# underactuated/HSLabs

Measured on AMD Instinct MI355X. Metric: batched control-loop steps/sec (hexapod.xml, 18-DoF) at 1/2/4/8 MI355X, higher is better.
Workload: dtype f64

## Files before the change

### hslabs_amd/api.py

```python
from __future__ import annotations

import ctypes
from dataclasses import dataclass, field

import numpy as np

from . import capi

GAIT_DTYPE = np.dtype([
    ("torso_pos", "<f8", (3,)), ("torso_angles", "<f8", (3,)), ("step_duration", "<f8"),
    ("period", "<f8"), ("step_length", "<f8"), ("step_height", "<f8"), ("curvature", "<f8"),
    ("foot_shift", "<f8"), ("foot_shift_type", "<i4"), ("rec_transform_flag", "<i4"),
    ("rec_transl", "<f8", (3,)), ("rec_eas", "<f8", (3,)), ("reserved", "<f8", (5,)),
])
assert GAIT_DTYPE.itemsize == 192


def _require(ok: bool, msg: str) -> None:
    if not ok:
        raise ValueError(msg)


def _torch_stream(device, stream):
    import torch
# ... 171 lines not shown
            pass


def limb_tile_launches() -> int:
    return int(capi.load().hs_limb_tile_launches())


def limb_tile_plan_launches() -> int:
    return int(capi.load().hs_limb_tile_plan_launches())


def limb_tile_loop_launches() -> int:
    return int(capi.load().hs_limb_tile_loop_launches())


def limb_launches() -> int:
    return int(capi.load().hs_limb_launches())


def limb_deferred() -> int:
    d = ctypes.c_int64()
    capi.check(capi.load().hs_limb_stats(None, ctypes.byref(d)), "hs_limb_stats")
    return int(d.value)


def params_array(params) -> np.ndarray:
    if isinstance(params, np.ndarray) and params.dtype == GAIT_DTYPE:
        return np.ascontiguousarray(params)
    arr = np.zeros(len(params), GAIT_DTYPE)
    for i, p in enumerate(params):
        arr[i] = p.to_record()
    return arr


def run_host(model: KinematicModel, params, n_t: int = 20, k0: int = 0, horizon: int | None = None,
             ignore_reach: bool = True, want=("q", "tau", "cf", "x", "flags", "work_cot")) -> dict:
    arr = params_array(params)
    B = len(arr)
    H = n_t if horizon is None else horizon
    shapes = _out_shapes(model, B, H)
    out = {k: np.zeros(shapes[k], np.uint32 if k == "flags" else np.float64) if k in want else None
           for k in ("q", "tau", "cf", "x", "flags", "work_cot")}
    dp = ctypes.POINTER(ctypes.c_double)

    def P(a, t=dp):
        return None if a is None else a.ctypes.data_as(t)
# ... 792 lines not shown
```

### hslabs_amd/capi.py

```python
from __future__ import annotations

import ctypes
import hashlib
import os

from . import build as _build

ABI_VERSION = 16

HS_OK = 0
HS_FLAG_RANK_RETRY = 1
HS_FLAG_FULL_RANK = 2
HS_FLAG_LOOP_EXHAUST = 4
HS_FLAG_NAN = 8
HS_FLAG_UNREACH = 16
HS_FLAG_NO_CONTACT = 32
HS_FLAG_GENERAL = 64
HS_FLAG_NEAR_RANK = 256
HS_FLAG_DEPENDENT = 512
HS_PREC_F64 = 0
HS_PREC_F32 = 1
HS_SOLVE_AUTO = 0
HS_SOLVE_REFERENCE = 1
KEY_MIN_STEP_LENGTH = 1e-3
COMM_ID_BYTES = 128

EXPORTS = [
    "hs_model_load", "hs_model_load_ex", "hs_model_free", "hs_model_get_dims", "hs_pgs_config_read",
    "hs_run", "hs_run_steps", "hs_run_calls", "hs_run_pd", "hs_run_forces", "hs_run_forces_calls", "hs_mixed_create", "hs_mixed_free",
    "hs_mixed_get_dims", "hs_complete_traj", "hs_traj_save", "hs_run_forces_host",
    "hs_run_mixed", "hs_run_mixed_steps", "hs_run_mixed_calls", "hs_run_host", "hs_best_key_cot", "hs_best_key_encode",
    "hs_best_key_decode", "hs_last_error", "hs_abi_version",
    "hs_sim_default_params", "hs_sim_reset", "hs_sim_step", "hs_sim_create", "hs_sim_advance", "hs_sim_get_state",
    "hs_sim_free", "hs_sim_trial", "hs_sim_trial_summary", "hs_sim_set_trial", "hs_sim_get_trial_state",
    "hs_sim_config", "hs_sim_track_push", "hs_sim_probe", "hs_sim_estimate_workspace",
    "hs_cpc_default_params", "hs_cpc_torques", "hs_cpc_target_points", "hs_sim_cpc_workspace", "hs_sim_cpc_step",
    "hs_batch_create", "hs_batch_set_params", "hs_batch_run", "hs_batch_run_device", "hs_select_best",
    "hs_batch_best_key_device", "hs_batch_free", "hs_comm_unique_id", "hs_comm_init", "hs_comm_free", "hs_comm_size",
    "hs_comm_reduce_best", "hs_select_best_comm", "hs_pergen_rec", "hs_pergen_rec_host", "hs_model_lik",
    "hs_model_lik_host", "hs_model_fk", "hs_model_fk_host", "hs_model_get_node", "hs_model_set_torso_penalty",
    "hs_model_get_torso_penalty", "hs_model_limb_lane", "hs_limb_launches", "hs_limb_tile_launches", "hs_limb_stats",
    "hs_limb_tile_plan_launches", "hs_limb_tile_loop_launches",
]
EXPORTS_B = ["hs_sim_regress_B", "hs_sim_estimate_B"]
HS_FLAG_LIK_FAILED = 128
SIM_BODY_STRIDE = 13
HS_TRIAL_RUNNING = -1
HS_TRIAL_SURVIVED = -2
HS_CPC_FLAG_NONFINITE = 1
HS_CPC_FLAG_NOSCORE = 2
HS_CPC_FLAG_RANK = 4


class GaitParamsC(ctypes.Structure):

    _fields_ = [
        ("torso_pos", ctypes.c_double * 3),
        ("torso_angles", ctypes.c_double * 3),
        ("step_duration", ctypes.c_double),
        ("period", ctypes.c_double),
        ("step_length", ctypes.c_double),
        ("step_height", ctypes.c_double),
        ("curvature", ctypes.c_double),
        ("foot_shift", ctypes.c_double),
        ("foot_shift_type", ctypes.c_int32),
# ... 236 lines not shown
    L.hs_batch_best_key_device.argtypes = [vp, ctypes.c_int32]
    L.hs_batch_best_key_device.restype = vp
    L.hs_batch_free.argtypes = [vp]
    L.hs_batch_free.restype = None
    u32p = ctypes.POINTER(ctypes.c_uint32)
    L.hs_pergen_rec.argtypes = [vp, vp, ctypes.c_int32, vp, ctypes.c_int32, vp, vp]
    L.hs_pergen_rec_host.argtypes = [vp, ctypes.POINTER(GaitParamsC), ctypes.c_int32, dp, ctypes.c_int32, dp]
    L.hs_model_lik.argtypes = [vp, ctypes.c_int32, vp, ctypes.c_int32, vp, vp, vp]
    L.hs_model_lik_host.argtypes = [vp, ctypes.c_int32, dp, ctypes.c_int32, dp, u32p]
    L.hs_model_fk.argtypes = [vp, ctypes.c_int32, vp, ctypes.c_int32, vp, vp, vp]
    L.hs_model_fk_host.argtypes = [vp, ctypes.c_int32, dp, ctypes.c_int32, dp, dp]
    L.hs_model_get_node.argtypes = [vp, ctypes.c_int32, ctypes.POINTER(NodeInfoC)]
    L.hs_last_error.argtypes = []
    L.hs_last_error.restype = ctypes.c_char_p
    L.hs_model_limb_lane.argtypes = [vp, ctypes.POINTER(ctypes.c_int32)]
    L.hs_limb_launches.argtypes = []
    L.hs_limb_launches.restype = ctypes.c_int64
    L.hs_limb_tile_launches.argtypes = []
    L.hs_limb_tile_launches.restype = ctypes.c_int64
    L.hs_limb_tile_plan_launches.argtypes = []
    L.hs_limb_tile_plan_launches.restype = ctypes.c_int64
    L.hs_limb_tile_loop_launches.argtypes = []
    L.hs_limb_tile_loop_launches.restype = ctypes.c_int64
    L.hs_limb_stats.argtypes = [ctypes.POINTER(ctypes.c_int64), ctypes.POINTER(ctypes.c_int64)]
    L.hs_abi_version.argtypes = []
    L.hs_abi_version.restype = ctypes.c_int
    if L.hs_abi_version() != ABI_VERSION:
        raise HSError("libhslabs ABI version mismatch")
    _lib = L
    return L


def check(rc: int, what: str = "") -> None:
    if rc != HS_OK:
        msg = load().hs_last_error().decode(errors="replace")
        raise HSError(f"{what}: {msg} (rc={rc})")
```

### hslabs_amd/csrc/hs_capi.cpp

```cpp
#include <hip/hip_runtime.h>

#include <algorithm>
#include <atomic>
#include <cmath>
#include <cstdio>
#include <cstdlib>
#include <cfloat>
#include <cstring>
#include <fstream>
#include <mutex>
#include <string>
#include <vector>

#include "hs_internal.h"

namespace {

thread_local std::string g_err;

int fail(int code, const std::string& msg) {
  g_err = msg;
  return code;
}

// ... 377 lines not shown
    std::lock_guard<std::mutex> lk(cx.pools->mu);
    hipError_t e = (hipError_t)cx.pools->fused_gen.get(
        a.stream, ((size_t)CHUNK * (B + 1) * hs::solve_workspace_bytes() + gwb - 1) / gwb, &gen);
    const size_t need = (size_t)S * B * sizeof(double);
    const size_t want =
        std::max(need, std::min((size_t)HS_FUSED_RESERVE_STEPS * B * sizeof(double), (size_t)512 << 20));
    if (e == hipSuccess) e = (hipError_t)cx.pools->fused_work.get(a.stream, (want + gwb - 1) / gwb, &work);
    if (e == hipSuccess)
      e = (hipError_t)cx.pools->fused_fix.get(a.stream, (fix_bytes(n_counts, CHUNK, mp) + gwb - 1) / gwb, &fix);
    if (e != hipSuccess) return hip_fail(e, "hipMalloc(fused workspace)");
  }
  int32_t* fix_counts = (int32_t*)fix;
  hs_run_args c = a;
  c.horizon = (int32_t)S;
  c.best_key = nullptr;
  hs_run_args r = a;
  if (r.key_steps == 0) r.key_steps = (int32_t)((int64_t)n_calls * a.horizon);
  mp.fused_h = a.horizon;
  mp.fused_work = work;
  mp.fused_gen = gen;
  fix_carve(fix, n_counts, mp);
  const bool barrier_ok = (B + 63) / 64 <= 1024 && env_switch("HS_FIX_BARRIER", true);
  mp.prep_unit = limb ? 8 : 2;
  int le = launch_setup(cx, c, mp);
  mp.red_total_mass = cx.total_mass;
  mp.red_rollout_mass = cx.rollout_mass;
  mp.red_key_steps = r.key_steps;
  hipStream_t st = (hipStream_t)a.stream;
  for (int32_t i = 0; le == 0 && i < n_chunks; i++) {
    const int64_t s0 = online ? 0 : (int64_t)i * CHUNK;
    const bool last = i + 1 == n_chunks;
    if (online) c.k0 = (int32_t)(((int64_t)a.k0 + (int64_t)i * a.horizon) % a.n_t);
    mp.fused_s0 = (int32_t)s0;
    mp.fused_n = (int32_t)std::min<int64_t>(CHUNK, S - s0);
    mp.fix_mode = hs::FIX_DEFER;
    mp.fix_count = fix_counts + i;
    mp.fix_reduce = 0;
    mp.limb_tile = limb_tile(rt, a, mp.fused_n);
    mp.limb_tile_loop = mp.limb_tile ? limb_tile_loop(a, mp.fused_n) : 1;
    hipError_t e = kernel_events ? hipEventRecord((hipEvent_t)kernel_events[2 * i], st) : hipSuccess;
    if (e != hipSuccess) return hip_fail(e, "hipEventRecord");
    int32_t planned = 0;
    le = limb ? k.launch_limb(cx.d_topo, c, cx.ws, mp, limb_tile_plan_mode(), &planned)
              : k.launch_fused(cx.d_topo, c, cx.ws, mp);
    g_limb_launches += limb;
    g_limb_tile_launches += mp.limb_tile;
// ... 36 lines not shown

int hs_abi_version(void) { return HSLABS_ABI_VERSION; }

int hs_model_limb_lane(hs_model_t m, int32_t* ok) {
  if (!m || !ok) return fail(HS_E_ARG, "null argument");
  *ok = m->host.limb_lane_ok;
  return HS_OK;
}

int64_t hs_limb_launches(void) { return g_limb_launches.load(); }
int64_t hs_limb_tile_launches(void) { return g_limb_tile_launches.load(); }
int64_t hs_limb_tile_plan_launches(void) { return g_limb_tile_plan_launches.load(); }
int64_t hs_limb_tile_loop_launches(void) { return g_limb_tile_loop_launches.load(); }

int hs_limb_stats(int64_t* launches, int64_t* deferred) {
  if (launches) *launches = g_limb_launches.load();
  if (deferred) {
    unsigned long long n[2] = {0, 0};
    hipError_t e = (hipError_t)hs::kernels_f64.limb_deferred(&n[0]);
    if (e == hipSuccess) e = (hipError_t)hs::kernels_f32.limb_deferred(&n[1]);
    if (e != hipSuccess) return hip_fail(e, "hs_limb_stats");
    *deferred = (int64_t)(n[0] + n[1]);
  }
  return HS_OK;
}

const char* hs_last_error(void) { return g_err.c_str(); }

int hs_model_load_ex(const char* xml_path, int lik_variant, hs_model_t* out) {
  if (!xml_path || !out) return fail(HS_E_ARG, "null argument");
  hs_model_s* m = new hs_model_s;
  memset(m->dev, 0, sizeof(m->dev));
  memset(m->sim_dev, 0, sizeof(m->sim_dev));
  memset(m->sim_dev_f32, 0, sizeof(m->sim_dev_f32));
  std::string err;
  int rc = hs::load_model_file(xml_path, lik_variant, &m->host, err, &m->sim);
  if (rc != HS_OK) {
    delete m;
    return fail(rc, err);
  }
  *out = m;
  return HS_OK;
}

int hs_model_load(const char* xml_path, hs_model_t* out) { return hs_model_load_ex(xml_path, -1, out); }

// ... 1597 lines not shown
```

### hslabs_amd/csrc/hs_internal.h

```cpp
#pragma once
#include <cstddef>
#include <mutex>
#include <string>
#include <vector>

#include "../../include/hslabs.h"
#include "hs_simtopo.h"
#include "hs_limb_tile.h"
#include "hs_topo.h"

struct hs_sim_probe_kargs {
  hs_sim_args sim;
  int32_t m, pad;
  const double* tau0;
  const double* dtau;
  double* config_out;
  double* tau_out;
  double* body_out;
  uint32_t* seed_out;
};

namespace hs {

int set_error(int code, const std::string& msg);
// ... 13 lines not shown
  int32_t n_waves;
  int32_t max_parts;
  int32_t h_row;
  int32_t setup_io;
  const double* tau_in;
  const double *pd_q, *pd_dq;
  double pd_k1, pd_k2;
  double *pd_tau, *pd_q0, *pd_dq0;
  int32_t st_tau, st_cf, st_q, st_x;
  int32_t fused_w, fused_s0, fused_n, fused_h;
  void* fused_work;
  void* fused_gen;
  int32_t setup_only;
  int32_t fix_mode;
  int32_t* fix_count;
  int32_t* fix_items;
  int32_t fix_n_counts;
  int32_t fix_reduce, red_key_steps, red_n_steps;
  int32_t* fix_barrier;
  double red_total_mass;
  const double* red_rollout_mass;
  uint64_t* red_best_key;
  int32_t ktab_n, ktab_lo, ktab_nl, ttab_n;
  int32_t prep_unit;
  const int32_t *limb_model, *limb_rollouts, *limb_slots;
  int32_t limb_waves;
  int32_t limb_tile;
  int32_t limb_tile_loop;
};

size_t solve_workspace_bytes();
void ktab_range(int32_t k0, int32_t n_t, int32_t horizon, int64_t n_calls, int32_t* lo, int32_t* n_table,
                int32_t* n_ttab);
launch_map single_model_map(const hs_topo& t, int32_t n_rollouts);

struct kernels {
  size_t (*general_workspace_bytes)();
  int (*launch_rollouts)(const hs_topo* d_topo, const hs_run_args& a, void* workspace, const launch_map& mp);
  int (*launch_fused)(const hs_topo* d_topo, const hs_run_args& a, void* workspace, const launch_map& mp);
  int (*launch_limb)(const hs_topo* d_topo, const hs_run_args& a, void* workspace, const launch_map& mp,
                     int32_t tile_plan, int32_t* tile_planned);
  int (*launch_fused_reduce)(const hs_run_args& a, double total_mass, const double* rollout_mass,
                             const void* work_steps, int32_t n_steps);
  int (*limb_deferred)(unsigned long long* out);
};
extern const kernels kernels_f64, kernels_f32;
inline const kernels& kernels_of(int32_t precision) { return precision == HS_PREC_F32 ? kernels_f32 : kernels_f64; }

int launch_pergen_rec(const hs_topo* d_topo, const hs_gait_params* params, int32_t n_rollouts, const double* times,
                      int32_t n_times, double* rec, void* stream);
int launch_fk(const hs_topo* d_topo, int32_t n_parts, int32_t n_cfg, const double* config, int32_t stride,
              double* a_ground, double* a_joint, void* stream);
int launch_lik(const hs_topo* d_topo, int32_t n_cfg, const double* rec, int32_t ignore_reach, double* config,
               uint32_t* status, void* stream);
// ... 65 lines not shown
```

### hslabs_amd/csrc/hs_kernels.hip

```cpp
#include "hs_rollout_kernel.h"
#include "hs_limb.h"

namespace {

__global__ __launch_bounds__(WAVE) void hs_pergen_rec_kernel(const hs_topo* __restrict__ T,
                                                             const hs_gait_params* __restrict__ params,
                                                             int32_t n_rollouts, const double* __restrict__ times,
                                                             int32_t n_times, double* __restrict__ rec) {
  __shared__ SetupL st[2];
  const int sub = threadIdx.x / HALF, lane = threadIdx.x % HALF;
  const int64_t n_items = (int64_t)n_rollouts * n_times;
  const int64_t item = (int64_t)blockIdx.x * 2 + sub;
  const bool live = item < n_items;
  const int64_t it = live ? item : n_items - 1;
  const int b = (int)(it / n_times), ti = (int)(it % n_times);
  const GaitR g = load_gait(params[b]);
  gait_setup(T, g, 1, st[sub], lane);
  const int nl = T->n_limbs;
  if (live && lane < nl) {
    real o0[3], o1[3], target[3];
    bool turned;
    gait_record<false>(g, params[b], limb_rec(st[sub], T->limb_pergen[lane]), (real)times[ti], o0, o1, turned, target);
    double* r = rec + it * (6 + 3 * nl);
    if (lane == 0)
// ... 13 lines not shown

#ifdef HS_STAMPS
extern "C" int hs_debug_read_stamps(unsigned long long* out, int n_rows) {
  if (n_rows > 4096) n_rows = 4096;
  return (int)hipMemcpyFromSymbol(out, HIP_SYMBOL(g_stamps), sizeof(unsigned long long) * 32 * n_rows, 0,
                                  hipMemcpyDeviceToHost);
}
extern "C" int hs_debug_set_stamp_base(unsigned int base) {
  return (int)hipMemcpyToSymbol(HIP_SYMBOL(g_stamp_base), &base, sizeof(base), 0, hipMemcpyHostToDevice);
}
extern "C" int hs_debug_set_stamp_iter(int iter) {
  return (int)hipMemcpyToSymbol(HIP_SYMBOL(g_stamp_iter), &iter, sizeof(iter), 0, hipMemcpyHostToDevice);
}
extern "C" int hs_debug_clear_stamps() {
  static unsigned long long zero[4096][32];
  return (int)hipMemcpyToSymbol(HIP_SYMBOL(g_stamps), zero, sizeof(zero), 0, hipMemcpyHostToDevice);
}
#endif

namespace hs {

size_t solve_workspace_bytes() { return sizeof(SolveWS); }

void ktab_range(int32_t k0, int32_t n_t, int32_t horizon, int64_t n_calls, int32_t* lo_out, int32_t* n_out,
                int32_t* ttab_out) {
  int64_t lo = INT64_MAX, hi = 0;
  const int64_t nc = n_calls < n_t ? n_calls : n_t;
  for (int64_t c = 0; c < nc; c++) {
    const int64_t f = ((int64_t)k0 + c * horizon) % n_t;
    lo = f < lo ? f : lo;
    hi = f + horizon + NS - 1 > hi ? f + horizon + NS - 1 : hi;
  }
  const int64_t n = nc > 0 ? hi - lo : 0;
  *lo_out = nc > 0 ? (int32_t)lo : 0;
  *n_out = n <= HS_KTAB ? (int32_t)n : 0;
  *ttab_out = (int32_t)(n < HS_KTAB ? n : HS_KTAB);
}

int launch_pergen_rec(const hs_topo* d_topo, const hs_gait_params* params, int32_t n_rollouts, const double* times,
                      int32_t n_times, double* rec, void* stream) {
  const int64_t items = (int64_t)n_rollouts * n_times;
  if (items <= 0) return 0;
  hipLaunchKernelGGL(hs_pergen_rec_kernel, dim3((unsigned)((items + 1) / 2)), dim3(WAVE), 0, (hipStream_t)stream,
                     d_topo, params, n_rollouts, times, n_times, rec);
  return (int)hipGetLastError();
}
// ... 8 lines not shown
```

### hslabs_amd/csrc/hs_limb.h

```cpp
#pragma once
#include "hs_limb_tile.h"
#include "hs_step_base.h"
#include "hs_step_kin.h"
#include "hs_step_solve.h"

namespace {

#ifndef HS_LIMB_WAVES
#define HS_LIMB_WAVES 2
#endif
#ifndef HS_LIMB_WAVES_F32
#define HS_LIMB_WAVES_F32 HS_LIMB_WAVES
#endif

constexpr int LG = 8;
constexpr int LGR = WAVE / LG;

__device__ inline int dbg_row(bool live, int b, int horizon, int s_glob) { return live ? b * horizon + s_glob : -1; }
#ifdef HS_DBG
#define LDBG(dbg_r, slot, val, n)                                                                                \
  do {                                                                                                           \
    if (HS_DBG == (n) && (dbg_r) >= 0 && (size_t)(dbg_r) * 32 + (slot) < (1u << 22)) g_dbg[(size_t)(dbg_r) * 32 + (slot)] = (double)(val); \
  } while (0)
#else
// ... 122 lines not shown
  return s;
}

__device__ __attribute__((always_inline)) inline A34 limb_frame(const hs_topo* T, int L, bool straight, const bool own,
                                                                const RolloutWS& W, const KinFrames& kf, int row,
                                                                const real* u, real tv, BodyS& ob) {
  if (straight) {
    if (own) ob = body_straight(kf.own[L][0], u, tv);
    return frame_at(load34r(kf.J0[L]), u, tv);
  }
  A34 A = load34r(W.ktor[row] + 6);
  const int clen = T->limb_chain_len[L];
  for (int kk = 1; kk < clen; kk++) {
    const int v = T->limb_chain[L][kk];
    A = mul(A, node_pj(T, v));
    if (T->node[v].owner_limb == L) {
      const real com[3] = {(real)T->node[v].com[0], (real)T->node[v].com[1], (real)T->node[v].com[2]};
      ob = body_frame(A, com);
    }
  }
  return mul(A, node_joint_parent(T, T->limb_child[L]));
}

__device__ inline bool sincos_big(real x) { return !(fabs(x) < (real)0x1p20); }
__device__ __attribute__((always_inline)) inline void limb_outer(const hs_topo* T, const hs_link (&LK)[3], const A34& J,
                                                                 const real* ja, real (&P)[3][3], real (&U)[3][3],
                                                                 bool& big) {
  real sq[3], cq[3];
#pragma unroll
  for (int kk = 0; kk < 3; kk++) {
    big |= sincos_big(ja[kk]);
    sincos_k_small(ja[kk], &sq[kk], &cq[kk]);
  }
  A34 Jv = J, H;
  real nul[3];
  bool nc = false;
#pragma unroll
  for (int kk = 0; kk < 3; kk++) fk_link<false>(T, LK[kk], kk, Jv, H, sq[kk], cq[kk], P[kk], U[kk], nul, nul, nul, nc);
}

__device__ __attribute__((always_inline)) inline void outer_put(real (&outer)[36][LGR * HS_LMAX], int o0, int col,
                                                                const real (&P)[3][3], const real (&U)[3][3]) {
#pragma unroll
  for (int kk = 0; kk < 3; kk++)
#pragma unroll
    for (int j = 0; j < 3; j++) {
      outer[o0 + 3 * kk + j][col] = P[kk][j];
      outer[o0 + 9 + 3 * kk + j][col] = U[kk][j];
    }
}
__device__ __attribute__((always_inline)) inline void outer_get(const real (&outer)[36][LGR * HS_LMAX], int kk, int col,
                                                                real* Pm, real* Um, real* Pp, real* Up) {
#pragma unroll
  for (int j = 0; j < 3; j++) {
    Pm[j] = outer[3 * kk + j][col];
    Um[j] = outer[9 + 3 * kk + j][col];
    Pp[j] = outer[18 + 3 * kk + j][col];
    Up[j] = outer[27 + 3 * kk + j][col];
  }
}

__device__ inline real wrap_rate(real q_plus, real q_minus, real dt) {
  const real dd = q_plus - q_minus;
  const real lo = dd - 2 * kPi, hi = dd + 2 * kPi;
  return (dd > kPi ? lo : (dd < -kPi ? hi : dd)) / (2 * dt);
}
__device__ inline bool limb_rows_big(const real* qm, const real* q0, const real* qp) {
  bool big = false;
#pragma unroll
  for (int kk = 0; kk < 3; kk++) big |= sincos_big(qm[kk]);
#pragma unroll
  for (int kk = 0; kk < 3; kk++) big |= sincos_big(q0[kk]);
#pragma unroll
  for (int kk = 0; kk < 3; kk++) big |= sincos_big(qp[kk]);
  return big;
}

__device__ inline void limb_defer(const hs::launch_map& mp, bool live, int l, int s_glob, int item) {
  if (l == 0 && live) {
    atomicAdd(&g_limb_deferred, 1ull);
    const int it = atomicAdd(mp.fix_count, 1);
    mp.fix_items[2 * it] = s_glob - mp.fused_s0;
    mp.fix_items[2 * it + 1] = item;
  }
}

__device__ inline int rank_limb(const hs_topo* T, uint32_t cm, int nl, int rank) {
  int src = 0;
  for (int L2 = 0; L2 < nl; L2++) {
// ... 234 lines not shown
  opaque_vals<3>(Jz);
  if (kk == 2) opaque_vals<3>(fp);
  real Pm[3], Um[3], Pp[3], Up[3];
  if constexpr (BARRIER) __builtin_amdgcn_sched_barrier(0);
  outer_get(outer, kk, ol, Pm, Um, Pp, Up);
  part_dyn(mk.mass(L, kk), inv, Pm, P0, Pp, Um, U0, Up, g);
  [[maybe_unused]] const int node = mk.node(L, kk);
  LDBG(dbg_r, node, P0[0], 1);
  LDBG(dbg_r, node, U0[0], 5);
  LDBG(dbg_r, node, g[0], 2);
  LDBG(dbg_r, node, g[3], 10);
  LDBG(dbg_r, node, g[1], 13);
  LDBG(dbg_r, node, g[2], 14);
  LDBG(dbg_r, node, g[4], 16);
  if (l == 0) LDBG(dbg_r, 31, o[0], 15);
  if (l == 0) LDBG(dbg_r, 30, o[1], 15);
  LDBG(dbg_r, node, Um[0], 9);
  LDBG(dbg_r, node, Up[0], 11);
  LDBG(dbg_r, node, Pm[0], 12);
  part_g(P0, o, g);
  LDBG(dbg_r, node, g[3], 3);
}

#ifdef HS_STAMPS
#undef HS_STAMP_GATE
#define HS_STAMP_GATE stamp_on
#endif
template <bool FORCES, bool LOOP>
__device__ __attribute__((always_inline)) inline void limb_tile_kd(
    const hs_topo* T_, const LimbModelK<LOOP>& mk, const KinFrames& kf, const real* ttab,
    real (&outer)[36][LGR * HS_LMAX], hs_link (&links)[HS_LMAX][3], const RolloutWS& W, bool straight,
    const real* u, real v, int lane, int nl, bool limb, int L, bool live, int row0, uint32_t M, uint64_t req,
    const real* tv, const real* o, real inv, real dt, LimbKD& kd, int dbg_r, bool stamp_on) {
  (void)dbg_r;
  (void)stamp_on;
  const int grp = lane >> 3, l = lane & 7;
  const bool shm = live && !((M >> (2 * grp)) & 1);
  const bool shp = live && !((M >> (2 * grp + 1)) & 1);
  const int nreq = __popc(M);
  auto nth_req = [req](int r) { return (int)(req >> (4 * r)) & 15; };
  const int nidle = LG - nl;
  const int E0 = (LGR * nidle) / nl;
  const int rqm = __popc(M & ((1u << (2 * grp)) - 1)), rqp = __popc(M & ((1u << (2 * grp + 1)) - 1));
  const int pm = shm || rqm < E0 ? 0 : 1 + (rqm - E0) / LGR, pp = shp || rqp < E0 ? 0 : 1 + (rqp - E0) / LGR;
  auto col = [](int ln) { return (ln >> 3) * HS_LMAX + (ln & 7); };
  real P[3][3], U[3][3];
  BodyS om, op, oc;
  kd.own = limb && mk.own(L);
  {
    int rq = 0, fL = L;
    bool extra = false;
    if (!limb) {
      const int j = grp * nidle + (l - nl);
      rq = j / nl;
      fL = j - rq * nl;
      extra = rq < E0 && rq < nreq;
      if (!extra) rq = 0, fL = 0;
    }
    const int bit = nth_req(rq), gr = bit >> 1, side = bit & 1;
    const int rr = __shfl(row0, gr * LG);
    const int frow = limb ? row0 + 2 : rr + 4 * side;
    const int dst = gr * LG + fL;
    const int dm = limb ? (shp ? lane + LG : -1) : (extra && side == 0 ? dst : -1);
    const int dp = limb ? (shm ? lane - LG : -1) : (extra && side == 1 ? dst : -1);
    BodyS ob;
#pragma unroll
    for (int j = 0; j < 3; j++) ob.P[j] = ob.U[j] = real(0);
    if (limb || extra) {
      const hs_topo* T = opaque_s(T_);
      const bool fown = LimbModelK<LOOP>{T, mk.k}.own(fL);
      const real tvf = LOOP && limb ? tv[2] : ttab[frow] * v;
// ... 31 lines not shown
#pragma unroll
    for (int j = 0; j < 3; j++) ob.P[j] = ob.U[j] = real(0);
    __builtin_amdgcn_sched_barrier(0);
    if (act) {
      real P2[3][3], U2[3][3];
      bool nb = false;
      const hs_topo* T = opaque_s(T_);
      limb_outer(T, links[L], limb_frame(T, L, straight, kd.own, W, kf, frow, u, ttab[frow] * v, ob), W.ktab[frow][L], P2,
                 U2, nb);
      outer_put(outer, side ? 18 : 0, col(dst), P2, U2);
    }
    if (!straight) {
#pragma unroll
      for (int j = 0; j < 6; j++) {
        const real val = j < 3 ? ob.P[j] : ob.U[j - 3];
        const real vm = lane_push(val, act && side == 0 ? dst : LG - 1), vp = lane_push(val, act && side == 1 ? dst : LG - 1);
        if (pm == pass) (j < 3 ? om.P[j] : om.U[j - 3]) = vm;
        if (pp == pass) (j < 3 ? op.P[j] : op.U[j - 3]) = vp;
      }
    }
  }
  __builtin_amdgcn_sched_barrier(0);
  STAMP(2);
  wave_sync();
  if (limb) {
    if (kd.own) {
      if (straight) {
        om = body_straight(kf.own[L][0], u, tv[0]);
        op = body_straight(kf.own[L][0], u, tv[4]);
      }
      part_dyn(mk.mass_own(L), inv, om.P, oc.P, op.P, om.U, oc.U, op.U, kd.gown);
      part_g(oc.P, o, kd.gown);
      if constexpr (FORCES)
        for (int j = 0; j < 3; j++) kd.Pown[j] = oc.P[j];
    }
    const int ol = grp * HS_LMAX + l;
#pragma unroll
    for (int kk = 0; kk < 3; kk++)
      limb_centre_link<FORCES, false>(mk, outer, ol, l, L, kk, P[kk], U[kk], kd.Jp[kk], kd.Jz[kk], kd.fp, kd.Pc[kk], o, inv, kd.g3[kk], dbg_r);
    kd.bad = W.kbad[row0 + 2][L] != 0;
    if constexpr (LOOP) {
      real jq[5][3];
#pragma unroll
      for (int r = 0; r < 5; r++)
#pragma unroll
        for (int kk = 0; kk < 3; kk++) jq[r][kk] = W.ktab[row0 + r][L][kk];
      kd.big |= limb_rows_big(jq[0], jq[2], jq[4]);
#pragma unroll
      for (int kk = 0; kk < 3; kk++) kd.jvel[kk] = wrap_rate(jq[3][kk], jq[1][kk], dt);
      return;
    }
    kd.big |= limb_rows_big(W.ktab[row0][L], W.ktab[row0 + 2][L], W.ktab[row0 + 4][L]);
#pragma unroll
    for (int kk = 0; kk < 3; kk++) {
      if constexpr (FORCES) break;
      kd.jvel[kk] = wrap_rate(W.ktab[row0 + 3][L][kk], W.ktab[row0 + 1][L][kk], dt);
    }
  }
}

template <bool FORCES>
__device__ __attribute__((always_inline)) inline void limb_packed_kd(
    const hs_topo* T_, real (&outer)[36][LGR * HS_LMAX], hs_link (&links)[HS_LMAX][3], const RolloutWS& W, bool straight,
    const real* u, int l, int L, int ol, int row, const real* tv, const real* o, real inv, real dt, LimbKD& kd, int dbg_r,
    bool stamp_on) {
  (void)stamp_on;
  kd.own = T_->limb_own_n[L] > 0;
  BodyS om, op, oc;
  {
    real P[3][3], U[3][3];
    const hs_topo* Ts = opaque_s(T_);
    limb_outer(Ts, links[L], limb_frame(Ts, L, straight, kd.own, W, W.kf, row, u, tv[0], om), W.ktab[row][L], P, U, kd.big);
    outer_put(outer, 0, ol, P, U);
  }
// ... 725 lines not shown
```

### hslabs_amd/csrc/hs_rollout_kernel.h

```cpp
#pragma once
#include "hs_step_base.h"
#include "hs_step_kin.h"
#include "hs_step_solve.h"

namespace {

template <bool DEFER, class W, class SV>
__device__ __attribute__((always_inline)) inline void step(const hs_topo* T, const hs_run_args& a, const hs::launch_map& mp, real dt, SV& sv,
                     FastL& fl, const W& w, SolveWS* G, int b, bool live, int h,
                     real& work, bool& deferred, bool may_general, int lane) {
  const int n = T->n, nmj = T->nmj, nf = T->nf, cfg = T->cfg, nl = T->n_limbs;
  STAMP(3);
  dynamics<false>(T, dt, sv, w, lane);
  STAMP(4);
  particular_sub(T, sv, w, lane);
  STAMP(5);
  const uint32_t cmask = half_ballot(lane < nf && w.contact(0, lane));
  const int nc = __popc(cmask);
  if (lane < nf && ((cmask >> lane) & 1)) sv.cfoot[__popc(cmask & ((1u << lane) - 1))] = lane;
  wave_sync();
  int k = 3 * nc;
  uint32_t flags = 0;
  STAMP(6);
  bool fast_near = false;
// ... 141 lines not shown
#endif
__device__ inline void wave_lds_sync() {
  __builtin_amdgcn_fence(__ATOMIC_SEQ_CST, "wavefront");
  __builtin_amdgcn_wave_barrier();
}
__device__ inline int ktab_lanes(const hs::launch_map& mp) { return mp.ktab_nl > 0 ? mp.ktab_nl : HS_LMAX; }
__host__ __device__ inline int prep_chunks(int ttab_n) { return (ttab_n > 0 ? ttab_n + HS_PREP_ROWS - 1 : HS_PREP_ROWS) / HS_PREP_ROWS; }
__host__ __device__ inline int prep_units(const hs::launch_map& mp, int n_rollouts, int& R) {
  R = mp.prep_unit > 2 && !mp.wave_rollouts ? mp.prep_unit : 2;
  return R == 2 ? mp.n_waves : (n_rollouts + R - 1) / R;
}
__host__ __device__ inline int64_t prep_blocks(int n_units, int R, int ttab_n, int nli) {
  const int64_t groups_per_xcd = R * (int64_t)prep_chunks(ttab_n) * ((n_units + 7) / 8);
  const int gpw = WAVE / nli;
  const int64_t waves_per_xcd = (groups_per_xcd + gpw - 1) / gpw;
  return 8 * ((waves_per_xcd + HS_PREP_WPB - 1) / HS_PREP_WPB);
}

template <bool MIXED>
__global__ __launch_bounds__(WAVE * HS_PREP_WPB, HS_PREP_WAVES) void hs_prep_kernel(const hs_topo* __restrict__ T0,
                                                                   hs_run_args a, RolloutWS* __restrict__ rws,
                                                                   hs::launch_map mp) {
  __shared__ real rad_s[HS_PREP_WPB][WAVE];
  __shared__ real q6s_s[HS_PREP_WPB][HS_PREP_ROWS][6][WAVE / 4];
  __shared__ real tgs_s[HS_PREP_WPB][HS_PREP_ROWS][3][WAVE];
  const int wv = (int)threadIdx.x / WAVE, tl = (int)threadIdx.x % WAVE;
  real(&rad)[WAVE] = rad_s[wv];
  real(&q6s)[HS_PREP_ROWS][6][WAVE / 4] = q6s_s[wv];
  real(&tgs)[HS_PREP_ROWS][3][WAVE] = tgs_s[wv];
  RSTAMP(29);
  STAMP(24);
  if (blockIdx.x == 0)
    for (int i = threadIdx.x; i < mp.fix_n_counts; i += blockDim.x) mp.fix_count[i] = 0;
  const int nli = ktab_lanes(mp), gpw = WAVE / nli;
  const int C = prep_chunks(mp.ttab_n);
  const int gl = tl / nli, L = tl % nli;
  const int gi = ((int)(blockIdx.x / 8) * HS_PREP_WPB + wv) * gpw + gl;
  int R;
  const int n_units = prep_units(mp, a.n_rollouts, R);
  const int chunk = gi % C, sub = (gi / C) % R, w = 8 * (gi / (R * C)) + (int)(blockIdx.x % 8);
  bool on = gl < gpw && w < n_units;
  int b = 0;
  const hs_topo* __restrict__ T = T0;
  if (on) {
    b = mp.wave_rollouts ? mp.wave_rollouts[2 * w + sub] : R * w + sub;
    if (MIXED) T = T0 + mp.wave_model[w];
    on = b >= 0 && b < a.n_rollouts && L < T->n_limbs;
  }
  GaitR g;
  A34 J0;
  real pos0[3], ts = 0, xs = 0, t_step = 0, dt = 0, v = 0;
  bool straight = false;
// ... 29 lines not shown
    }
    if (g.curvature != 0) my_rad = turn_radius(pos0, g.curvature);
  }
  STAMP(25);
  rad[tl] = my_rad;
  wave_lds_sync();
  real mr = 0;
  if (on && g.curvature != 0)
    for (int l = 0; l < T->n_limbs; l++) {
      const real r = rad[tl - L + l];
      if (r > mr) mr = r;
    }
  if (on && chunk == 0 && L == 0) ws->st.max_radius = mr;
  STAMP(26);
  if (!on) return;
  const int r0 = chunk * HS_PREP_ROWS, r1 = min(r0 + HS_PREP_ROWS, mp.ttab_n);
  if (r0 >= r1) return;
  const bool table = mp.ktab_n > 0;
  const hs_aff34& Jp0 = T->node[0].J_A_parent;
  const real u[3] = {(real)Jp0.m[0], (real)Jp0.m[1], (real)Jp0.m[2]};
  const real ls[3] = {(real)T->ls[0], (real)T->ls[1], (real)T->ls[2]};
  const int kind = T->lik_kind;
  const bool ir = a.ignore_reach != 0;
  auto store_row = [&](int r, const real* ja, bool bad) {
    real* e = ws->ktab[r][L];
#pragma unroll
    for (int kk = 0; kk < 3; kk++) e[kk] = ja[kk];
    ws->kbad[r][L] = bad ? 1 : 0;
  };
  real t = sample_time_sum(dt, mp.ktab_lo + r0);
  if (!table || straight) {
#pragma unroll 1
    for (int r = r0; r < r1; r++) {
      if (r > r0) t += dt;
      if (L == 0) ws->t_tab[r] = t;
      if (table) {
        real dx, dz;
        limb_step(g, t, ts, xs, t_step, dx, dz);
        const real target[3] = {dx + pos0[0], real(0) + pos0[1], dz + pos0[2]};
        real ja[3];
        bool bad;
        hip_ik_k(frame_at(J0, u, t * v), target, kind, ls, plan.ysign, ir, ja, bad);
        store_row(r, ja, bad);
      }
      if (r == r0) STAMP(27);
    }
  } else {
    const LimbRec rl{v, t_step, mr, ts, xs, {pos0[0], pos0[1], pos0[2]}, tsc};
    const hs_gait_params& gp = a.params[b];
#pragma unroll 1
    for (int r = r0; r < r1; r++) {
      if (r > r0) t += dt;
      if (L == 0) ws->t_tab[r] = t;
      real o0[3], o1[3], target[3];
      bool turned;
      gait_record<false>(g, gp, rl, t, o0, o1, turned, target);
      if (L == 0) {
        const real q6[6] = {o0[0], o0[1], o0[2], o1[0], o1[1], o1[2]};
        for (int i = 0; i < 6; i++) q6s[r - r0][i][gl] = q6[i];
      }
      for (int i = 0; i < 3; i++) tgs[r - r0][i][tl] = target[i];
    }
    wave_lds_sync();
#pragma unroll 1
    for (int r = r0; r < r1; r++) {
      real q6[6], target[3];
      for (int i = 0; i < 6; i++) q6[i] = q6s[r - r0][i][gl];
      for (int i = 0; i < 3; i++) target[i] = tgs[r - r0][i][tl];
      const A34 A0 = mul(mul(node_joint_parent(T, 0), free_joint(q6)), node_pj(T, 0));
      if (L == 0) {
        real* tr = ws->ktor[r];
        for (int i = 0; i < 6; i++) tr[i] = q6[i];
        store34r(A0, tr + 6);
      }
      A34 A = A0;
      for (int k = 1; k < T->limb_chain_len[L]; k++) A = mul(A, node_pj(T, T->limb_chain[L][k]));
      real ja[3];
      bool bad;
      hip_ik(T, L, mul(A, node_joint_parent(T, T->limb_child[L])), target, ir, ja, bad);
      store_row(r, ja, bad);
      if (r == r0) STAMP(27);
    }
  }
  STAMP(28);
  RSTAMP(30);
}

template <int NM, bool FORCES, bool DEFER>
__device__ __attribute__((always_inline)) inline void rollout_wave(const hs_topo* __restrict__ T0, const hs_run_args& a,
                                                                   RolloutWS* __restrict__ rws, const hs::launch_map& mp,
                                                                   Smem<NM, FORCES>* smem, int fstep, int wid,
                                                                   int only_sub) {
  const int sub = threadIdx.x / HALF;
  const int lane = threadIdx.x % HALF;
  const hs_topo* __restrict__ T = mp.wave_model ? T0 + mp.wave_model[wid] : T0;
  int b, bb;
  bool live;
  if (mp.wave_rollouts) {
    b = mp.wave_rollouts[2 * wid + sub];
    live = b >= 0;
    bb = live ? b : mp.wave_rollouts[2 * wid];
  } else {
    b = wid * 2 + sub;
    live = b < a.n_rollouts;
// ... 255 lines not shown
```

### hslabs_amd/csrc/hs_step_base.h

```cpp
#pragma once
#include <hip/hip_runtime.h>

#include <cfloat>
#include <cstdint>
#include <type_traits>

#ifndef HS_REAL_IS_FLOAT
#define HS_REAL_IS_FLOAT 0
#endif
#include "hs_internal.h"
#include "hs_math.h"

namespace {

using namespace hsd;

#ifndef HS_CURVED_LDS
#define HS_CURVED_LDS HS_REAL_IS_FLOAT
#endif
#ifndef HS_PRELOAD
#define HS_PRELOAD (!HS_REAL_IS_FLOAT)
#endif
#ifndef HS_KTE_PRELOAD
#define HS_KTE_PRELOAD (!HS_REAL_IS_FLOAT)
// ... 234 lines not shown
  __device__ bool want_q(int k) const { return k >= -1 && k <= 1; }
  __device__ bool want_centre(int k) const { return k == 0; }
  __device__ real* pos(int k, int v) const { return k == 0 ? d->c.pos[v] : d->sten.pos[k > 0][v]; }
  __device__ real* ust(int k, int v) const { return d->sten.ust[(k + 2) >> 1][v]; }
  __device__ real* q(int k) const { return d->c.q[k + 1]; }
  __device__ real* jpos(int, int v) const { return d->c.jpos[v]; }
  __device__ real* jz(int, int v) const { return d->c.jz[v]; }
  __device__ real* fpos(int, int f) const { return d->c.fpos[f]; }
  __device__ int& contact(int, int f) const { return d->c.contact[f]; }
  __device__ int& unreach(int, int L) const { return d->c.unreach[L]; }
};

#ifndef HS_KTAB
#define HS_KTAB 64
#endif
struct RolloutWS {
  SolveWS sol;
  SetupL st;
  real t_tab[HS_KTAB];
  KinFrames kf;
  real ktab[HS_KTAB][HS_LMAX][KT_W];
  real ktor[HS_KTAB][KR_W];
  uint8_t kbad[HS_KTAB][HS_LMAX];
};
static_assert(sizeof(SetupL) % sizeof(real) == 0, "SetupL is copied as reals");

constexpr int kFusedGroup = 256;
__device__ inline void fused_coords(int blk, int W, int n, int& fstep, int& wid) {
  const int q = blk / (kFusedGroup * n), g0 = q * kFusedGroup;
  const int gw = W - g0 < kFusedGroup ? W - g0 : kFusedGroup;
  const int r = blk - g0 * n;
  fstep = r / gw;
  wid = g0 + r % gw;
}

}

namespace hs {

template <class F>
inline void with_lds_class(int max_parts, F&& f) {
  if (max_parts <= 18) f(std::integral_constant<int, 18>{});
  else if (max_parts <= 22) f(std::integral_constant<int, 22>{});
  else f(std::integral_constant<int, HS_NMAX>{});
}

// ... 2 lines not shown
```

### hslabs_amd/csrc/hs_step_kin.h

```cpp
#pragma once
#include "hs_step_base.h"

namespace {

struct GaitR {
  real torso_pos[3], torso_angles[3];
  real step_duration, period, step_length, step_height, curvature, foot_shift;
  int foot_shift_type;
  int rec_xf;
};

__device__ inline GaitR load_gait(const hs_gait_params& p) {
  GaitR g;
  for (int i = 0; i < 3; i++) {
    g.torso_pos[i] = (real)p.torso_pos[i];
    g.torso_angles[i] = (real)p.torso_angles[i];
  }
  g.step_duration = (real)p.step_duration;
  g.period = (real)p.period;
  g.step_length = (real)p.step_length;
  g.step_height = (real)p.step_height;
  g.curvature = (real)p.curvature;
  g.foot_shift = (real)p.foot_shift;
  g.foot_shift_type = p.foot_shift_type;
// ... 263 lines not shown
    real sg, cg;
    sincos(gamma, &sg, &cg);
    dx = r * sg * sb;
    dy += -r * cg * sb;
  }
  target[0] = dx + st.pos0[0];
  target[1] = dy + st.pos0[1];
  target[2] = dz + st.pos0[2];
  if (!STRAIGHT && g.rec_xf) {
    transform_rec(gp, o0, o1, target);
    turned = true;
  }
}

__device__ inline real sample_time_sum(real dt, int isample) {
  real t = 0;
  for (int i = 0; i < isample; i++) t += dt;
  return t;
}
__device__ inline real sample_time(const SetupL& st, const real* t_tab, int isample, int lo, int ttab_n) {
  const int r = isample - lo;
  if (t_tab && r >= 0 && r < ttab_n) return t_tab[r];
  return sample_time_sum(st.dt, isample);
}

template <class W>
__device__ __attribute__((always_inline)) inline void limb_fk(const hs_topo* T, int L, const A34& J, const real* ja,
                                                              const real* sq, const real* cq, bool wq, const W& w,
                                                              int k) {
  const int lv[3] = {T->limb_node[L][0], T->limb_node[L][1], T->limb_node[L][2]};
  A34 Jv = J, H;
#pragma unroll
  for (int kk = 0; kk < 3; kk++) {
    const hs_link& lk = T->link[L][kk];
    if (kk > 0) Jv = mul(H, load34(lk.P));
    H = mul_hinge(Jv, cq[kk], sq[kk]);
    if (wq) w.q(k)[6 + lk.hinge] = ja[kk];
    const int v = lv[kk];
    if (w.want_pos(k)) {
      const real c[3] = {(real)lk.com[0], (real)lk.com[1], (real)lk.com[2]};
      real p[3];
      mulp(H, c, p);
      real* P = w.pos(k, v);
      for (int i = 0; i < 3; i++) P[i] = p[i];
      if (k == 0) DBG(v, p[0], 1);
      if (k == -2) DBG(v, p[0], 12);
// ... 407 lines not shown
```

### include/hslabs.h

```cpp
#ifndef HSLABS_H
#define HSLABS_H
#include <stddef.h>
#include <stdint.h>
#ifdef __cplusplus
extern "C" {
#endif

#define HSLABS_ABI_VERSION 16

enum {
  HS_OK = 0,
  HS_E_ARG = -1,
  HS_E_IO = -2,
  HS_E_PARSE = -3,
  HS_E_TOPOLOGY = -4,
  HS_E_NOLIK = -5,
  HS_E_DEVICE = -6,
  HS_E_NOTFOUND = -7
};

#define HS_FLAG_RANK_RETRY   1u
#define HS_FLAG_FULL_RANK    2u
#define HS_FLAG_LOOP_EXHAUST 4u
#define HS_FLAG_NAN          8u
// ... 361 lines not shown
} hs_sim_cpc_args;

size_t hs_sim_cpc_workspace(hs_model_t model, int32_t n_rollouts, int32_t m);

int hs_sim_cpc_step(hs_model_t model, const hs_sim_cpc_args* args);

typedef struct hs_sim_s* hs_sim_t;
int hs_sim_create(hs_model_t model, const hs_gait_params* params, int32_t n_rollouts, const hs_sim_params* sim_params,
                  double t0, hs_sim_t* out);
int hs_sim_advance(hs_sim_t sim, int32_t n_steps, double* tau_cmd, double* q_meas, double* torso, int32_t* n_contacts,
                   double* normal_force);
int hs_sim_get_state(hs_sim_t sim, double* body, int32_t* tsi);
int hs_sim_set_trial(hs_sim_t sim, int32_t open_loop, double torque_limit, int32_t kick_every, int32_t kick_phase,
                     const double* kick_dv_host, double hc, int32_t check_from, int32_t check_until);
int hs_sim_get_trial_state(hs_sim_t sim, int32_t* state_host);
void hs_sim_free(hs_sim_t sim);

int hs_model_limb_lane(hs_model_t model, int32_t* ok);
int64_t hs_limb_launches(void);
int64_t hs_limb_tile_launches(void);
int64_t hs_limb_tile_plan_launches(void);
int64_t hs_limb_tile_loop_launches(void);
int hs_limb_stats(int64_t* launches, int64_t* deferred);

const char* hs_last_error(void);
int hs_abi_version(void);

#ifdef __cplusplus
}
#endif
#endif
```

Measured before the change: 1.063 billion.

## Precompute limb joint rates and big flags in setup kernel tables

The setup/prep kernel now computes, for each table row, the wrapped central-difference joint velocity and the large-angle flag. It does this by evaluating one extra halo row per wave and exchanging neighbour rows through LDS, then stores the results into new kvel/kbig arrays in the rollout workspace. The tiled loop kernel reads these precomputed values, issued early before a wave sync, instead of loading five ktab rows and computing wrap_rate per step. The cost is extra IK work for halo rows, a larger workspace and more LDS. A debug readback API for the tables is also added.

```diff
diff --git a/hslabs_amd/api.py b/hslabs_amd/api.py
--- a/hslabs_amd/api.py
+++ b/hslabs_amd/api.py
@@ -217,6 +217,17 @@
     d = ctypes.c_int64()
     capi.check(capi.load().hs_limb_stats(None, ctypes.byref(d)), "hs_limb_stats")
     return int(d.value)
+
+
+def limb_tables(model, rollout: int, n_rows: int, device=None, stream=None) -> dict:
+    out = dict(ktab=np.zeros((n_rows, 6, 3)), kvel=np.zeros((n_rows, 6, 3)), kbig=np.zeros((n_rows, 6), np.uint8),
+               kbad=np.zeros((n_rows, 6), np.uint8))
+    dt = ctypes.c_double()
+    capi.check(capi.load().hs_debug_limb_tables(model.handle, _cuda_stream(device, stream), rollout, n_rows,
+                                                *(out[k].ctypes.data for k in ("ktab", "kvel", "kbig", "kbad")),
+                                                ctypes.addressof(dt)), "hs_debug_limb_tables")
+    out["dt"] = float(dt.value)
+    return out
 
 
 def params_array(params) -> np.ndarray:
diff --git a/hslabs_amd/capi.py b/hslabs_amd/capi.py
--- a/hslabs_amd/capi.py
+++ b/hslabs_amd/capi.py
@@ -40,7 +40,7 @@
     "hs_comm_reduce_best", "hs_select_best_comm", "hs_pergen_rec", "hs_pergen_rec_host", "hs_model_lik",
     "hs_model_lik_host", "hs_model_fk", "hs_model_fk_host", "hs_model_get_node", "hs_model_set_torso_penalty",
     "hs_model_get_torso_penalty", "hs_model_limb_lane", "hs_limb_launches", "hs_limb_tile_launches", "hs_limb_stats",
-    "hs_limb_tile_plan_launches", "hs_limb_tile_loop_launches",
+    "hs_limb_tile_plan_launches", "hs_limb_tile_loop_launches", "hs_debug_limb_tables",
 ]
 EXPORTS_B = ["hs_sim_regress_B", "hs_sim_estimate_B"]
 HS_FLAG_LIK_FAILED = 128
@@ -323,6 +323,8 @@
     L.hs_limb_tile_plan_launches.restype = ctypes.c_int64
     L.hs_limb_tile_loop_launches.argtypes = []
     L.hs_limb_tile_loop_launches.restype = ctypes.c_int64
+    L.hs_debug_limb_tables.argtypes = [vp, vp, ctypes.c_int32, ctypes.c_int32, vp, vp, vp, vp, vp]
+    L.hs_debug_limb_tables.restype = ctypes.c_int
     L.hs_limb_stats.argtypes = [ctypes.POINTER(ctypes.c_int64), ctypes.POINTER(ctypes.c_int64)]
     L.hs_abi_version.argtypes = []
     L.hs_abi_version.restype = ctypes.c_int
diff --git a/hslabs_amd/csrc/hs_capi.cpp b/hslabs_amd/csrc/hs_capi.cpp
--- a/hslabs_amd/csrc/hs_capi.cpp
+++ b/hslabs_amd/csrc/hs_capi.cpp
@@ -423,6 +423,9 @@
   fix_carve(fix, n_counts, mp);
   const bool barrier_ok = (B + 63) / 64 <= 1024 && env_switch("HS_FIX_BARRIER", true);
   mp.prep_unit = limb ? 8 : 2;
+  mp.ktab_rates = 0;
+  for (int32_t i = 0; !online && i < n_chunks; i++)
+    mp.ktab_rates |= limb_tile(rt, a, (int32_t)std::min<int64_t>(CHUNK, S - (int64_t)i * CHUNK)) ? 1 : 0;
   int le = launch_setup(cx, c, mp);
   mp.red_total_mass = cx.total_mass;
   mp.red_rollout_mass = cx.rollout_mass;
@@ -505,6 +508,24 @@
     if (e != hipSuccess) return hip_fail(e, "hs_limb_stats");
     *deferred = (int64_t)(n[0] + n[1]);
   }
+  return HS_OK;
+}
+
+int hs_debug_limb_tables(hs_model_t m, void* stream, int32_t rollout, int32_t n_rows, double* ktab, double* kvel,
+                         uint8_t* kbig, uint8_t* kbad, double* dt) {
+  if (!m) return fail(HS_E_ARG, "null argument");
+  int dev = 0;
+  hipError_t e = hipGetDevice(&dev);
+  if (e != hipSuccess) return hip_fail(e, "hipGetDevice");
+  const void* ws = nullptr;
+  {
+    std::lock_guard<std::mutex> lk(m->mu);
+    for (const auto& s : m->ws.live)
+      if (s.dev == dev && s.stream == stream && rollout >= 0 && (size_t)rollout < s.n) ws = s.ptr;
+  }
+  if (!ws) return fail(HS_E_ARG, "no workspace of this model, device and stream holds that rollout");
+  e = (hipError_t)hs::limb_tables_read(ws, rollout, n_rows, ktab, kvel, kbig, kbad, dt, stream);
+  if (e != hipSuccess) return hip_fail(e, "hs_debug_limb_tables");
   return HS_OK;
 }
 
diff --git a/hslabs_amd/csrc/hs_internal.h b/hslabs_amd/csrc/hs_internal.h
--- a/hslabs_amd/csrc/hs_internal.h
+++ b/hslabs_amd/csrc/hs_internal.h
@@ -59,6 +59,7 @@
   const double* red_rollout_mass;
   uint64_t* red_best_key;
   int32_t ktab_n, ktab_lo, ktab_nl, ttab_n;
+  int32_t ktab_rates = 0;
   int32_t prep_unit;
   const int32_t *limb_model, *limb_rollouts, *limb_slots;
   int32_t limb_waves;
@@ -67,6 +68,8 @@
 };
 
 size_t solve_workspace_bytes();
+int limb_tables_read(const void* workspace, int32_t rollout, int32_t n_rows, double* ktab, double* kvel, uint8_t* kbig,
+                     uint8_t* kbad, double* dt, void* stream);
 void ktab_range(int32_t k0, int32_t n_t, int32_t horizon, int64_t n_calls, int32_t* lo, int32_t* n_table,
                 int32_t* n_ttab);
 launch_map single_model_map(const hs_topo& t, int32_t n_rollouts);
diff --git a/hslabs_amd/csrc/hs_kernels.hip b/hslabs_amd/csrc/hs_kernels.hip
--- a/hslabs_amd/csrc/hs_kernels.hip
+++ b/hslabs_amd/csrc/hs_kernels.hip
@@ -59,6 +59,23 @@
 
 size_t solve_workspace_bytes() { return sizeof(SolveWS); }
 
+int limb_tables_read(const void* workspace, int32_t rollout, int32_t n_rows, double* ktab, double* kvel, uint8_t* kbig,
+                     uint8_t* kbad, double* dt, void* stream) {
+  static_assert(std::is_same<real, double>::value, "the fp64 unit's RolloutWS");
+  if (n_rows < 0 || n_rows > HS_KTAB) return (int)hipErrorInvalidValue;
+  const RolloutWS* W = (const RolloutWS*)workspace + rollout;
+  hipError_t e = hipStreamSynchronize((hipStream_t)stream);
+  const auto get = [&](void* dst, const void* src, size_t n) {
+    if (e == hipSuccess && dst && n) e = hipMemcpy(dst, src, n, hipMemcpyDeviceToHost);
+  };
+  get(ktab, W->ktab, sizeof(W->ktab[0]) * n_rows);
+  get(kvel, W->kvel, sizeof(W->kvel[0]) * n_rows);
+  get(kbig, W->kbig, sizeof(W->kbig[0]) * n_rows);
+  get(kbad, W->kbad, sizeof(W->kbad[0]) * n_rows);
+  get(dt, &W->st.dt, sizeof(double));
+  return (int)e;
+}
+
 void ktab_range(int32_t k0, int32_t n_t, int32_t horizon, int64_t n_calls, int32_t* lo_out, int32_t* n_out,
                 int32_t* ttab_out) {
   int64_t lo = INT64_MAX, hi = 0;
diff --git a/hslabs_amd/csrc/hs_limb.h b/hslabs_amd/csrc/hs_limb.h
--- a/hslabs_amd/csrc/hs_limb.h
+++ b/hslabs_amd/csrc/hs_limb.h
@@ -168,7 +168,6 @@
   return mul(A, node_joint_parent(T, T->limb_child[L]));
 }
 
-__device__ inline bool sincos_big(real x) { return !(fabs(x) < (real)0x1p20); }
 __device__ __attribute__((always_inline)) inline void limb_outer(const hs_topo* T, const hs_link (&LK)[3], const A34& J,
                                                                  const real* ja, real (&P)[3][3], real (&U)[3][3],
                                                                  bool& big) {
@@ -206,11 +205,6 @@
   }
 }
 
-__device__ inline real wrap_rate(real q_plus, real q_minus, real dt) {
-  const real dd = q_plus - q_minus;
-  const real lo = dd - 2 * kPi, hi = dd + 2 * kPi;
-  return (dd > kPi ? lo : (dd < -kPi ? hi : dd)) / (2 * dt);
-}
 __device__ inline bool limb_rows_big(const real* qm, const real* q0, const real* qp) {
   bool big = false;
 #pragma unroll
@@ -491,6 +485,26 @@
   LDBG(dbg_r, node, g[3], 3);
 }
 
+struct LimbTileRates {
+  real v[3];
+  uint32_t big0, big2, big4, bad;
+  __device__ __attribute__((always_inline)) inline void issue(const RolloutWS& W, int row0, int L) {
+#pragma unroll
+    for (int kk = 0; kk < 3; kk++) v[kk] = W.kvel[row0 + 2][L][kk];
+    big0 = W.kbig[row0][L];
+    big2 = W.kbig[row0 + 2][L];
+    big4 = W.kbig[row0 + 4][L];
+    bad = W.kbad[row0 + 2][L];
+  }
+  __device__ __attribute__((always_inline)) inline void finish(LimbKD& kd) {
+    asm volatile("" : "+v"(big0), "+v"(big2), "+v"(big4), "+v"(bad));
+    kd.bad = bad != 0;
+    kd.big |= (big0 | big2 | big4) != 0;
+#pragma unroll
+    for (int kk = 0; kk < 3; kk++) kd.jvel[kk] = v[kk];
+  }
+};
+
 #ifdef HS_STAMPS
 #undef HS_STAMP_GATE
 #define HS_STAMP_GATE stamp_on
@@ -516,6 +530,7 @@
   real P[3][3], U[3][3];
   BodyS om, op, oc;
   kd.own = limb && mk.own(L);
+  [[maybe_unused]] LimbTileRates tr;
   {
     int rq = 0, fL = L;
     bool extra = false;
@@ -593,6 +608,8 @@
   }
   __builtin_amdgcn_sched_barrier(0);
   STAMP(2);
+  if constexpr (LOOP)
+    if (limb) tr.issue(W, row0, L);
   wave_sync();
   if (limb) {
     if (kd.own) {
@@ -609,18 +626,11 @@
 #pragma unroll
     for (int kk = 0; kk < 3; kk++)
       limb_centre_link<FORCES, false>(mk, outer, ol, l, L, kk, P[kk], U[kk], kd.Jp[kk], kd.Jz[kk], kd.fp, kd.Pc[kk], o, inv, kd.g3[kk], dbg_r);
+    if constexpr (LOOP) {
+      tr.finish(kd);
+      return;
+    }
     kd.bad = W.kbad[row0 + 2][L] != 0;
-    if constexpr (LOOP) {
-      real jq[5][3];
-#pragma unroll
-      for (int r = 0; r < 5; r++)
-#pragma unroll
-        for (int kk = 0; kk < 3; kk++) jq[r][kk] = W.ktab[row0 + r][L][kk];
-      kd.big |= limb_rows_big(jq[0], jq[2], jq[4]);
-#pragma unroll
-      for (int kk = 0; kk < 3; kk++) kd.jvel[kk] = wrap_rate(jq[3][kk], jq[1][kk], dt);
-      return;
-    }
     kd.big |= limb_rows_big(W.ktab[row0][L], W.ktab[row0 + 2][L], W.ktab[row0 + 4][L]);
 #pragma unroll
     for (int kk = 0; kk < 3; kk++) {
diff --git a/hslabs_amd/csrc/hs_rollout_kernel.h b/hslabs_amd/csrc/hs_rollout_kernel.h
--- a/hslabs_amd/csrc/hs_rollout_kernel.h
+++ b/hslabs_amd/csrc/hs_rollout_kernel.h
@@ -187,12 +187,12 @@
                                                                    hs_run_args a, RolloutWS* __restrict__ rws,
                                                                    hs::launch_map mp) {
   __shared__ real rad_s[HS_PREP_WPB][WAVE];
-  __shared__ real q6s_s[HS_PREP_WPB][HS_PREP_ROWS][6][WAVE / 4];
-  __shared__ real tgs_s[HS_PREP_WPB][HS_PREP_ROWS][3][WAVE];
+  __shared__ real q6s_s[HS_PREP_WPB][HS_PREP_ROWS + 1][6][WAVE / 4];
+  __shared__ real tgs_s[HS_PREP_WPB][HS_PREP_ROWS + 1][3][WAVE];
   const int wv = (int)threadIdx.x / WAVE, tl = (int)threadIdx.x % WAVE;
   real(&rad)[WAVE] = rad_s[wv];
-  real(&q6s)[HS_PREP_ROWS][6][WAVE / 4] = q6s_s[wv];
-  real(&tgs)[HS_PREP_ROWS][3][WAVE] = tgs_s[wv];
+  real(&q6s)[HS_PREP_ROWS + 1][6][WAVE / 4] = q6s_s[wv];
+  real(&tgs)[HS_PREP_ROWS + 1][3][WAVE] = tgs_s[wv];
   RSTAMP(29);
   STAMP(24);
   if (blockIdx.x == 0)
@@ -268,7 +268,16 @@
   const real ls[3] = {(real)T->ls[0], (real)T->ls[1], (real)T->ls[2]};
   const int kind = T->lik_kind;
   const bool ir = a.ignore_reach != 0;
-  auto store_row = [&](int r, const real* ja, bool bad) {
+  const int n = r1 - r0;
+  const bool rates = table && mp.ktab_rates != 0;
+  const int hrow = !rates ? -1 : (gl == 0 && r0 > 0 ? r0 - 1 : (gl == gpw - 1 && r1 < mp.ttab_n ? r1 : -1));
+  const int nit = n + (__any(hrow >= 0) ? 1 : 0);
+  auto store_row = [&](int slot, int r, const real* ja, bool bad) {
+    if (rates) {
+#pragma unroll
+      for (int kk = 0; kk < 3; kk++) tgs[slot][kk][tl] = ja[kk];
+    }
+    if (slot == HS_PREP_ROWS) return;
     real* e = ws->ktab[r][L];
 #pragma unroll
     for (int kk = 0; kk < 3; kk++) e[kk] = ja[kk];
@@ -277,9 +286,13 @@
   real t = sample_time_sum(dt, mp.ktab_lo + r0);
   if (!table || straight) {
 #pragma unroll 1
-    for (int r = r0; r < r1; r++) {
-      if (r > r0) t += dt;
-      if (L == 0) ws->t_tab[r] = t;
+    for (int it = 0; it < nit; it++) {
+      const bool mine = it < n;
+      const int r = mine ? r0 + it : hrow, slot = mine ? it : HS_PREP_ROWS;
+      if (r < 0) continue;
+      if (!mine) t = sample_time_sum(dt, mp.ktab_lo + r);
+      else if (it > 0) t += dt;
+      if (L == 0 && mine) ws->t_tab[r] = t;
       if (table) {
         real dx, dz;
         limb_step(g, t, ts, xs, t_step, dx, dz);
@@ -287,34 +300,41 @@
         real ja[3];
         bool bad;
         hip_ik_k(frame_at(J0, u, t * v), target, kind, ls, plan.ysign, ir, ja, bad);
-        store_row(r, ja, bad);
-      }
-      if (r == r0) STAMP(27);
+        store_row(slot, r, ja, bad);
+      }
+      if (it == 0) STAMP(27);
     }
   } else {
     const LimbRec rl{v, t_step, mr, ts, xs, {pos0[0], pos0[1], pos0[2]}, tsc};
     const hs_gait_params& gp = a.params[b];
 #pragma unroll 1
-    for (int r = r0; r < r1; r++) {
-      if (r > r0) t += dt;
-      if (L == 0) ws->t_tab[r] = t;
+    for (int it = 0; it < nit; it++) {
+      const bool mine = it < n;
+      const int r = mine ? r0 + it : hrow, slot = mine ? it : HS_PREP_ROWS;
+      if (r < 0) continue;
+      if (!mine) t = sample_time_sum(dt, mp.ktab_lo + r);
+      else if (it > 0) t += dt;
+      if (L == 0 && mine) ws->t_tab[r] = t;
       real o0[3], o1[3], target[3];
       bool turned;
       gait_record<false>(g, gp, rl, t, o0, o1, turned, target);
       if (L == 0) {
         const real q6[6] = {o0[0], o0[1], o0[2], o1[0], o1[1], o1[2]};
-        for (int i = 0; i < 6; i++) q6s[r - r0][i][gl] = q6[i];
-      }
-      for (int i = 0; i < 3; i++) tgs[r - r0][i][tl] = target[i];
+        for (int i = 0; i < 6; i++) q6s[slot][i][gl] = q6[i];
+      }
+      for (int i = 0; i < 3; i++) tgs[slot][i][tl] = target[i];
     }
     wave_lds_sync();
 #pragma unroll 1
-    for (int r = r0; r < r1; r++) {
+    for (int it = 0; it < nit; it++) {
+      const bool mine = it < n;
+      const int r = mine ? r0 + it : hrow, slot = mine ? it : HS_PREP_ROWS;
+      if (r < 0) continue;
       real q6[6], target[3];
-      for (int i = 0; i < 6; i++) q6[i] = q6s[r - r0][i][gl];
-      for (int i = 0; i < 3; i++) target[i] = tgs[r - r0][i][tl];
+      for (int i = 0; i < 6; i++) q6[i] = q6s[slot][i][gl];
+      for (int i = 0; i < 3; i++) target[i] = tgs[slot][i][tl];
       const A34 A0 = mul(mul(node_joint_parent(T, 0), free_joint(q6)), node_pj(T, 0));
-      if (L == 0) {
+      if (L == 0 && mine) {
         real* tr = ws->ktor[r];
         for (int i = 0; i < 6; i++) tr[i] = q6[i];
         store34r(A0, tr + 6);
@@ -324,8 +344,32 @@
       real ja[3];
       bool bad;
       hip_ik(T, L, mul(A, node_joint_parent(T, T->limb_child[L])), target, ir, ja, bad);
-      store_row(r, ja, bad);
-      if (r == r0) STAMP(27);
+      store_row(slot, r, ja, bad);
+      if (it == 0) STAMP(27);
+    }
+  }
+  if (rates) {
+    wave_lds_sync();
+    real qm[3] = {0, 0, 0}, q0[3], qp[3] = {0, 0, 0};
+    const bool lane_m = hrow == r0 - 1, lane_p = hrow == r1;
+    if (r0 > 0)
+      for (int kk = 0; kk < 3; kk++) qm[kk] = lane_m ? tgs[HS_PREP_ROWS][kk][tl] : tgs[HS_PREP_ROWS - 1][kk][tl - nli];
+    for (int kk = 0; kk < 3; kk++) q0[kk] = tgs[0][kk][tl];
+#pragma unroll 1
+    for (int it = 0; it < n; it++) {
+      const int r = r0 + it;
+      const bool next = r + 1 < mp.ttab_n;
+      if (next)
+        for (int kk = 0; kk < 3; kk++)
+          qp[kk] = it + 1 < n ? tgs[it + 1][kk][tl] : (lane_p ? tgs[HS_PREP_ROWS][kk][tl] : tgs[0][kk][tl + nli]);
+      bool big = false;
+      for (int kk = 0; kk < 3; kk++) big |= sincos_big(q0[kk]);
+      ws->kbig[r][L] = big ? 1 : 0;
+      if (r > 0 && next) {
+        real* e = ws->kvel[r][L];
+        for (int kk = 0; kk < 3; kk++) e[kk] = wrap_rate(qp[kk], qm[kk], dt);
+      }
+      for (int kk = 0; kk < 3; kk++) qm[kk] = q0[kk], q0[kk] = qp[kk];
     }
   }
   STAMP(28);
diff --git a/hslabs_amd/csrc/hs_step_base.h b/hslabs_amd/csrc/hs_step_base.h
--- a/hslabs_amd/csrc/hs_step_base.h
+++ b/hslabs_amd/csrc/hs_step_base.h
@@ -280,6 +280,8 @@
   real ktab[HS_KTAB][HS_LMAX][KT_W];
   real ktor[HS_KTAB][KR_W];
   uint8_t kbad[HS_KTAB][HS_LMAX];
+  real kvel[HS_KTAB][HS_LMAX][KT_W];
+  uint8_t kbig[HS_KTAB][HS_LMAX];
 };
 static_assert(sizeof(SetupL) % sizeof(real) == 0, "SetupL is copied as reals");
 
diff --git a/hslabs_amd/csrc/hs_step_kin.h b/hslabs_amd/csrc/hs_step_kin.h
--- a/hslabs_amd/csrc/hs_step_kin.h
+++ b/hslabs_amd/csrc/hs_step_kin.h
@@ -309,6 +309,13 @@
   const int r = isample - lo;
   if (t_tab && r >= 0 && r < ttab_n) return t_tab[r];
   return sample_time_sum(st.dt, isample);
+}
+
+__device__ inline bool sincos_big(real x) { return !(fabs(x) < (real)0x1p20); }
+__device__ inline real wrap_rate(real q_plus, real q_minus, real dt) {
+  const real dd = q_plus - q_minus;
+  const real lo = dd - 2 * kPi, hi = dd + 2 * kPi;
+  return (dd > kPi ? lo : (dd < -kPi ? hi : dd)) / (2 * dt);
 }
 
 template <class W>
diff --git a/include/hslabs.h b/include/hslabs.h
--- a/include/hslabs.h
+++ b/include/hslabs.h
@@ -407,6 +407,8 @@
 int64_t hs_limb_tile_plan_launches(void);
 int64_t hs_limb_tile_loop_launches(void);
 int hs_limb_stats(int64_t* launches, int64_t* deferred);
+int hs_debug_limb_tables(hs_model_t model, void* stream, int32_t rollout, int32_t n_rows, double* ktab, double* kvel,
+                         uint8_t* kbig, uint8_t* kbad, double* dt);
 
 const char* hs_last_error(void);
 int hs_abi_version(void);
```

After: 1.088 billion, median of 6. +2.4%, better.
